# SonyResearch/micro_diffusion

Measured on AMD Instinct MI355X. Metric: training images/sec (global batch 2048) MicroDiT-XL/2 256-res mask=0.75, higher is better.
Workload: dtype bf16; 1 GPU; MicroDiT_XL_2 res_256_pretrain.yaml mask=0.75, full step = 2 microbatches x 1024 fwd+bwd + grad exchange + clip 0.25 + AdamW; global_batch=2048, microbatch=1024, parallelism=dp1, grad_exchange=none (single rank)

## Files before the change

### micro_diffusion_amd/csrc/gemm.hip

```cpp
#include "md_common.h"
#include "gemm_common.h"
#include <stdlib.h>

namespace {

constexpr int BM = 128, BN = 128;
constexpr int PITCH_KC = (BKT + 8) * 2;
constexpr int PITCH_KS = (BM + 32) * 2;
constexpr int TILE_BYTES = (BM * PITCH_KC > BKT * PITCH_KS) ? BM * PITCH_KC : BKT * PITCH_KS;
constexpr int SLAB_PITCH = 68;
constexpr int SLAB_FLOATS = 32 * SLAB_PITCH;
static_assert(4 * SLAB_FLOATS * 4 <= 2 * TILE_BYTES, "epilogue slab must fit in the staging LDS");

typedef __attribute__((address_space(3))) s16x4 lds_s16x4;

__device__ __forceinline__ bf16x4 lds_tr_read(const unsigned char* p) {
    s16x4 v = __builtin_amdgcn_ds_read_tr16_b64_v4i16((lds_s16x4*)(p));
    U64 t;
    t.s = v;
    return t.h;
}

__device__ __forceinline__ void tile_coords(int bid, int nwg, int ntn, int group_n, int& tm, int& tn) {
    const int q = nwg >> 3, r = nwg & 7, xcd = bid & 7, j = bid >> 3;
// ... 366 lines not shown
    long long* const tl = static_cast<long long*>(p.timeline);
    timeline_stamp(tl, 0);
    const int64_t m0 = (int64_t)tile_m * TM;
    const int64_t n0 = (int64_t)tile_n * TN;
    const int batch = blockIdx.y / p.ksplit;
    const int split = blockIdx.y % p.ksplit;
    const bf16* A = reinterpret_cast<const bf16*>(p.A) + (int64_t)batch * p.sA;
    const bf16* B = reinterpret_cast<const bf16*>(p.B) + (int64_t)batch * p.sB;
    const int64_t ntk = (p.K + BKT - 1) / BKT;
    const int64_t tps = (ntk + p.ksplit - 1) / p.ksplit;
    const int64_t kbeg = (int64_t)split * tps * BKT;
    int64_t kend = kbeg + tps * BKT;
    if (kend > p.K) kend = p.K;
    const int nt = kbeg < kend ? (int)((kend - kbeg + BKT - 1) / BKT) : 0;

    f32x16 acc[MI][2];
#pragma unroll
    for (int i = 0; i < MI; ++i)
#pragma unroll
        for (int j = 0; j < 2; ++j)
#pragma unroll
            for (int r = 0; r < 16; ++r) acc[i][j][r] = 0.f;

    const unsigned lds0 = (unsigned)(uintptr_t)(lds_void_t*)smem;
    if (nt > 0) {
        dma_tile<AKC, TM>(smem, A, p.lda, m0, p.M, kbeg, kend, wave, lane);
        dma_tile<BKC, TN>(smem + ATILE, B, p.ldb, n0, p.N, kbeg, kend, wave, lane);
    }
    bf16x8 fa[2][MI], fb[2][2];
    for (int t = 0; t < nt; ++t) {
        const int cur = t & 1;
        const bool more = t + 1 < nt;
        const int64_t k0 = kbeg + (int64_t)(t + 1) * BKT;
        unsigned char* nb = smem + (cur ^ 1) * BUF;
        if (PACED) {
            asm volatile("s_waitcnt vmcnt(0)" ::: "memory");
            __builtin_amdgcn_s_barrier();
        } else {
            if (more) {
                dma_tile<AKC, TM>(nb, A, p.lda, m0, p.M, k0, kend, wave, lane);
                dma_tile<BKC, TN>(nb + ATILE, B, p.ldb, n0, p.N, k0, kend, wave, lane);
                asm volatile("s_waitcnt vmcnt(8)" ::: "memory");
            } else {
                asm volatile("s_waitcnt vmcnt(0)" ::: "memory");
            }
            __builtin_amdgcn_s_barrier();
        }
        if (t == 0) timeline_stamp(tl, 1);
        const unsigned sA = lds0 + cur * BUF, sB = sA + ATILE;
#pragma unroll
        for (int i = 0; i < MI; ++i) fa[0][i] = dma_frag<AKC, TM>(sA, wm * (MI * 32) + i * 32, 0, lane);
#pragma unroll
        for (int j = 0; j < 2; ++j) fb[0][j] = dma_frag<BKC, TN>(sB, wn * 64 + j * 32, 0, lane);
        asm volatile("s_waitcnt lgkmcnt(0)" ::: "memory");
#pragma unroll
        for (int ks = 0; ks < BKT / 16; ++ks) {
            const int cb = ks & 1, nx = cb ^ 1;
            if (PACED && more) {
                dma_tile<AKC, TM>(nb, A, p.lda, m0, p.M, k0, kend, wave, lane, ks, ks + 1);
                dma_tile<BKC, TN>(nb + ATILE, B, p.ldb, n0, p.N, k0, kend, wave, lane, ks, ks + 1);
            }
            if (ks + 1 < BKT / 16) {
#pragma unroll
                for (int i = 0; i < MI; ++i) fa[nx][i] = dma_frag<AKC, TM>(sA, wm * (MI * 32) + i * 32, ks + 1, lane);
#pragma unroll
                for (int j = 0; j < 2; ++j) fb[nx][j] = dma_frag<BKC, TN>(sB, wn * 64 + j * 32, ks + 1, lane);
            }
            __builtin_amdgcn_sched_barrier(0);
#pragma unroll
            for (int i = 0; i < MI; ++i)
#pragma unroll
                for (int j = 0; j < 2; ++j)
                    acc[i][j] = __builtin_amdgcn_mfma_f32_32x32x16_bf16(fa[cb][i], fb[cb][j], acc[i][j], 0, 0, 0);
            __builtin_amdgcn_sched_barrier(0);
            if (ks + 1 < BKT / 16) asm volatile("s_waitcnt lgkmcnt(0)" ::: "memory");
            __builtin_amdgcn_sched_barrier(0);
        }
        if (!PACED) __builtin_amdgcn_s_barrier();
    }
    if (PACED) __builtin_amdgcn_s_barrier();
    timeline_stamp(tl, 2);
    gemm_epilogue<MI>(p, acc, smem, m0 + wm * (MI * 32), n0 + wn * 64, batch, split, wave, lane);
    timeline_finish(tl);
}

__device__ __forceinline__ float4 nt_ld4(const float* p) {
    const f32x4 v = __builtin_nontemporal_load(reinterpret_cast<const f32x4*>(p));
    return make_float4(v[0], v[1], v[2], v[3]);
}
__global__ __launch_bounds__(256) void splitk_reduce_kernel(const float* ws, float* out, int64_t M, int64_t N, int64_t ldo,
                                                            int64_t sOut, int ksplit, int batch, int accumulate, int64_t slice) {
    const int64_t n4 = N / 4, per = M * n4, total = per * batch;
    for (int64_t i = (int64_t)blockIdx.x * 256 + threadIdx.x; i < total; i += (int64_t)gridDim.x * 256) {
        const int64_t b = i / per, r = i % per, m = r / n4, c = (r % n4) * 4;
        const float* src = ws + (b * ksplit) * slice + m * N + c;
        float4 acc = make_float4(0.f, 0.f, 0.f, 0.f);
        int s = 0;
        for (; s + 4 <= ksplit; s += 4) {
            const float4 v0 = nt_ld4(src + (int64_t)s * slice), v1 = nt_ld4(src + (int64_t)(s + 1) * slice);
            const float4 v2 = nt_ld4(src + (int64_t)(s + 2) * slice), v3 = nt_ld4(src + (int64_t)(s + 3) * slice);
            acc.x += (v0.x + v1.x) + (v2.x + v3.x); acc.y += (v0.y + v1.y) + (v2.y + v3.y);
            acc.z += (v0.z + v1.z) + (v2.z + v3.z); acc.w += (v0.w + v1.w) + (v2.w + v3.w);
        }
        for (; s < ksplit; ++s) {
            const float4 v = nt_ld4(src + (int64_t)s * slice);
            acc.x += v.x; acc.y += v.y; acc.z += v.z; acc.w += v.w;
        }
        if (accumulate == 2) {
            bf16x4 o;
            o[0] = f2bf(acc.x); o[1] = f2bf(acc.y); o[2] = f2bf(acc.z); o[3] = f2bf(acc.w);
            st_bf16x4(reinterpret_cast<bf16*>(out) + b * sOut + m * ldo + c, o);
            continue;
        }
        float* dst = out + b * sOut + m * ldo + c;
        if (accumulate) {
            const float4 o = *reinterpret_cast<const float4*>(dst);
            acc.x += o.x; acc.y += o.y; acc.z += o.z; acc.w += o.w;
        }
        *reinterpret_cast<float4*>(dst) = acc;
    }
}

}

extern "C" int md_splitk_reduce(const float* ws, float* out, int64_t M, int64_t N, int64_t ldo, int64_t sOut, int32_t ksplit,
                                int32_t batch, int32_t accumulate, hipStream_t stream) {
    if (!ws || !out || M <= 0 || N <= 0 || N % 4 || ldo % 4 || ksplit <= 0 || batch <= 0 || accumulate < 0 || accumulate > 2) return MD_BAD_ARG;
    int64_t grid = (M * (N / 4) * batch + 255) / 256;
    if (grid > 16384) grid = 16384;
    hipLaunchKernelGGL(splitk_reduce_kernel, dim3((unsigned)grid), dim3(256), 0, stream, ws, out, M, N, ldo, sOut, ksplit, batch,
                       accumulate, M * N);
    MD_LAUNCH_CHECK();
    return 0;
}

extern "C" int md_splitk_reduce_flat(const float* ws, float* out, int64_t n, int64_t slice_stride, int32_t ksplit, int32_t accumulate,
                                     hipStream_t stream) {
    if (!ws || !out || n <= 0 || n % 4 || slice_stride < n || slice_stride % 4 || ksplit <= 0 || accumulate < 0 || accumulate > 2) return MD_BAD_ARG;
    int64_t grid = (n / 4 + 255) / 256;
    if (grid > 16384) grid = 16384;
    hipLaunchKernelGGL(splitk_reduce_kernel, dim3((unsigned)grid), dim3(256), 0, stream, ws, out, (int64_t)1, n, n, (int64_t)0, ksplit, 1,
                       accumulate, slice_stride);
    MD_LAUNCH_CHECK();
    return 0;
}

static bool md_gemm_w4_fills(int64_t tiles, int cu_limit) {
    if (!(cu_limit > 0 && cu_limit < 256)) return true;
    if (tiles <= cu_limit) return false;
    const int64_t rounds = (tiles + cu_limit - 1) / cu_limit;
    return tiles * 100 >= rounds * cu_limit * 92;
}

extern "C" int md_gemm_bf16(const md_gemm_args* a_in, hipStream_t stream) {
    if (!a_in) return MD_BAD_ARG;
    md_gemm_args a_copy = *a_in;
    const md_gemm_args* a = &a_copy;
    if (a->problems) {
        if (!a->C || a->K <= 0 || a->ksplit <= 0 || a->mode != MD_EPI_STORE_F32 || a->sSplit <= 0 || !md_gemm_pp_eligible(a)) return MD_BAD_ARG;
        if (a->variant != MD_GEMM_AUTO && a->variant != MD_GEMM_PP256 && a->variant != MD_GEMM_W4) return MD_NOT_ELIGIBLE;
        if (a->variant == MD_GEMM_W4 && !md_gemm_w4_eligible(a)) return MD_NOT_ELIGIBLE;
        bool w4 = a->variant == MD_GEMM_W4;
        if (a->variant == MD_GEMM_AUTO && md_gemm_w4_eligible(a) && !getenv("MD_GEMM_NO_W4") && !getenv("MD_GEMM_NO_W4_TN")) {
            int64_t t = 0;
            for (int i = 0; i < a->n_problems; ++i) t += ((a->problems[i].M + 255) / 256) * ((a->problems[i].N + 255) / 256);
            w4 = md_gemm_w4_fills(t * a->ksplit, a->cu_limit);
        }
        if (a->chosen_variant) *a->chosen_variant = w4 ? MD_GEMM_W4 : MD_GEMM_PP256;
        return w4 ? md_gemm_w4_launch(a, stream) : md_gemm_pp_launch(a, stream);
    }
    if (!a->A || !a->B || !a->C) return MD_BAD_ARG;
    if (a->M <= 0 || a->N <= 0 || a->K <= 0 || a->batch <= 0 || a->ksplit <= 0) return MD_BAD_ARG;
    if (a->lda % 8 || a->ldb % 8) return MD_BAD_ARG;
    if ((a->mode == MD_EPI_STORE_BF16 || a->mode == MD_EPI_RESIDUAL || a->mode == MD_EPI_DACT || a->mode == MD_EPI_SWIGLU_BWD) ? (a->ldc % 8) : (a->ldc % 4))
        return MD_BAD_ARG;
    if (a->C2 && a->ldc2 % 8) return MD_BAD_ARG;
    if (a->ksplit > 1 && !(a->mode == MD_EPI_ATOMIC_F32 || (a->mode == MD_EPI_STORE_F32 && a->sSplit > 0))) return MD_BAD_ARG;
    if (a->mode == MD_EPI_RESIDUAL && (!a->res || (a->gate && a->rows_per_sample <= 0))) return MD_BAD_ARG;
    if (a->mode == MD_EPI_DACT && !a->aux) return MD_BAD_ARG;
    if (a->mode < MD_EPI_STORE_BF16 || a->mode > MD_EPI_SWIGLU_BWD) return MD_BAD_ARG;
    if (a->mode == MD_EPI_SWIGLU_BWD) {
        if (!a->aux || a->ldaux % 8) return MD_BAD_ARG;
        if (a->variant != MD_GEMM_AUTO && a->variant != MD_GEMM_W4) return MD_NOT_ELIGIBLE;
        if (!md_gemm_w4_eligible(a) || (a->cu_limit > 0 && a->cu_limit < 256) || getenv("MD_GEMM_NO_W4")) return MD_NOT_ELIGIBLE;
        a_copy.variant = MD_GEMM_W4;
    }
    if (a->dact_cached && (a->act != MD_ACT_GELU_ERF || !(a->mode == MD_EPI_DACT || (a->mode == MD_EPI_STORE_BF16 && a->C2)))) return MD_BAD_ARG;
    const int64_t tiles256 = ((a->M + 255) / 256) * ((a->N + 255) / 256) * (int64_t)a->batch * a->ksplit;
    const int64_t kspan = (a->K + a->ksplit - 1) / a->ksplit;
    int variant = a->variant;
    if (variant < MD_GEMM_AUTO || variant > MD_GEMM_W4) return MD_BAD_ARG;
    if (variant == MD_GEMM_PP256 && !md_gemm_pp_eligible(a)) return MD_NOT_ELIGIBLE;
    if (variant == MD_GEMM_W4 && !md_gemm_w4_eligible(a)) return MD_NOT_ELIGIBLE;
    if ((a->A_list || a->B_list) && !(a->A_list && a->B_list && md_gemm_pp_eligible(a))) return MD_BAD_ARG;
    if (a->A_list) variant = MD_GEMM_PP256;
    if (variant == MD_GEMM_AUTO) {
        const char* w4min = getenv("MD_GEMM_W4_MIN_TILES");
        if (md_gemm_w4_eligible(a) && tiles256 >= (w4min ? atoi(w4min) : 192) && md_gemm_w4_fills(tiles256, a->cu_limit) && !getenv("MD_GEMM_NO_W4") &&
            (a->a_kcontig || !getenv("MD_GEMM_NO_W4_TN")))
            variant = MD_GEMM_W4;
        else if (md_gemm_pp_eligible(a) && tiles256 >= 192)
            variant = MD_GEMM_PP256;
        else if (!a->a_kcontig && !a->b_kcontig && kspan >= 2048 && tiles256 >= 128)
            variant = MD_GEMM_PACED256;
        else if (a->K >= 1024 && tiles256 >= 224 && tiles256 <= 256)
            variant = MD_GEMM_PACED256;
        else if (kspan > 2048 && tiles256 >= 240 && (tiles256 % 256 == 0 || tiles256 % 256 >= 160 || tiles256 >= 2048))
            variant = MD_GEMM_PACED256;
        else if (a->a_kcontig && a->K <= 2048)
            variant = MD_GEMM_REG128;
        else
            variant = ((!a->a_kcontig && !a->b_kcontig) || a->K < 1024) ? MD_GEMM_REG128 : MD_GEMM_DMA128;
    }
    const int TMv = variant >= MD_GEMM_PACED256 ? 256 : 128;
    if (a->raster_group_n <= 0) {
        const int64_t ntn_ = (a->N + TMv - 1) / TMv;
        int64_t g = (2 << 20) / (TMv * kspan * 2);
        if (variant >= MD_GEMM_PP256 && g < 4) g = 4;
        if (g < 1) g = 1;
        if (g > ntn_) g = ntn_;
        a_copy.raster_group_n = (int)g;
    }
    if (a->chosen_variant) *a->chosen_variant = variant;
    if (variant == MD_GEMM_W4) return md_gemm_w4_launch(a, stream);
    if (variant >= MD_GEMM_PP256) return md_gemm_pp_launch(a, stream);
    const int64_t tiles = ((a->M + TMv - 1) / TMv) * ((a->N + TMv - 1) / TMv);
    dim3 grid((unsigned)tiles, (unsigned)(a->batch * a->ksplit), 1);
#define LAUNCH(KERN, THREADS, ...)                                                                                          \
    do {                                                                                                                   \
        if (a->a_kcontig && a->b_kcontig) hipLaunchKernelGGL((KERN<1, 1 __VA_ARGS__>), grid, dim3(THREADS), 0, stream, *a);       \
        else if (a->a_kcontig && !a->b_kcontig) hipLaunchKernelGGL((KERN<1, 0 __VA_ARGS__>), grid, dim3(THREADS), 0, stream, *a); \
        else if (!a->a_kcontig && a->b_kcontig) hipLaunchKernelGGL((KERN<0, 1 __VA_ARGS__>), grid, dim3(THREADS), 0, stream, *a); \
        else hipLaunchKernelGGL((KERN<0, 0 __VA_ARGS__>), grid, dim3(THREADS), 0, stream, *a);                                     \
    } while (0)
#define COMMA ,
    if (variant == MD_GEMM_REG128) LAUNCH(gemm_bf16_kernel, 256, );
    else if (variant == MD_GEMM_DMA128) LAUNCH(gemm_bf16_dma_kernel, 256, COMMA 2 COMMA 2 COMMA 2);
    else LAUNCH(gemm_bf16_dma_kernel, 512, COMMA 2 COMMA 4 COMMA 4 COMMA true);
#undef COMMA
#undef LAUNCH
    MD_LAUNCH_CHECK();
    return 0;
}
```

### micro_diffusion_amd/csrc/gemm_w4.hip

```cpp
#include "gemm_pp_common.h"

namespace {

struct W4Addr {
    unsigned adA[8];
    unsigned adB[8];
    unsigned aofs[8], bofs[8];
    unsigned ldsw;
};

#ifndef W4_ACC_INC
#define W4_ACC_INC "gemm_w4_acc.inc"
#endif
#include W4_ACC_INC

constexpr int W4_BUF = 32768;
constexpr int W4_BREG = 65536;
constexpr int W4_SLAB = 8192;

constexpr bool w4_is_dact(int epi) { return epi == PP_E_DACT_GELU || epi == PP_E_DACT_MUL || epi == PP_E_DACT_SWIGLU; }



typedef unsigned w4_u32x2 __attribute__((ext_vector_type(2), may_alias));
typedef unsigned w4_u32x4 __attribute__((ext_vector_type(4), may_alias));

struct W4Tile {
    int m0, n0, batch;
    int mlim, nlim;
    char* cbase;
    char* c2base;
    const char* opbase;
    const char* gbase;
};

struct W4EpiLane {
    unsigned wr[8];
    unsigned rd[4];
    unsigned oc, oc2, oo, og;
    int rg, c8;
};
struct W4Ops {
    uint4 v[4];
    uint4 gq;
    uint4 v2[4];
};

template <int EPI>
__device__ __forceinline__ void w4_epi_lane(const md_gemm_args& p, const W4Tile& et, int wcol, int lane_in, W4EpiLane& L) {
    int lane = lane_in;
    asm volatile("" : "+v"(lane));
    const int r = lane & 15, g = lane >> 4;
#pragma unroll
    for (int j = 0; j < 8; ++j) L.wr[j] = (unsigned)(r * 256 + ((32 * j + 8 * g) ^ (r << 4)));
#pragma unroll
    for (int t = 0; t < 4; ++t) L.rd[t] = (unsigned)((4 * t + g) * 256 + ((16 * r) ^ ((4 * t + g) << 4)));
    L.rg = g;
    L.c8 = r * 8;
    const int cc = wcol + r * 8 < et.nlim ? r * 8 : 0;
    L.oc = (unsigned)(g * (int)p.ldc + r * 8) * 2u;
    L.oc2 = (unsigned)(g * (int)p.ldc2 + r * 8) * 2u;
    L.oo = (unsigned)(g * (int)(EPI == PP_E_RES ? p.ldr : p.ldaux) + cc) * 2u;
    L.og = (unsigned)cc * 2u;
}

struct W4Rows {
    char* c;
    char* c2;
    const char* op;
    int64_t sc, sc2, so;
};

template <int EPI, bool INTERIOR>
__device__ __forceinline__ void w4_epi_req(const md_gemm_args& p, const W4Tile& et, const W4EpiLane& L, const char* oprow, int row0, int wcol, uint4& dst) {
    if (INTERIOR) {
        dst = *reinterpret_cast<const uint4*>(oprow + L.oo);
    } else if constexpr (EPI == PP_E_DACT_SWIGLU) {
        dst = make_uint4(0u, 0u, 0u, 0u);
    } else {
        const int64_t ldo = EPI == PP_E_RES ? p.ldr : p.ldaux;
        const int row = row0 + L.rg < et.mlim - 1 ? row0 + L.rg : et.mlim - 1;
        dst = *reinterpret_cast<const uint4*>(et.opbase + ((int64_t)row * ldo + wcol) * 2 + L.og);
    }
}
template <int EPI, int I>
__device__ __forceinline__ void w4_epi_gate(const md_gemm_args& p, const PPPlan& w, const W4Tile& et, const W4EpiLane& L, int wrow, int wcol, uint4& gq) {
    gq = make_uint4(0x3f803f80u, 0x3f803f80u, 0x3f803f80u, 0x3f803f80u);
    if (et.gbase) {
        int r0 = et.m0 + wrow + 16 * I;
        r0 = r0 < w.M - 1 ? r0 : w.M - 1;
        const unsigned srow = w.rps_shift >= 0 ? (unsigned)r0 >> w.rps_shift : (unsigned)r0 / (unsigned)p.rows_per_sample;
        gq = *reinterpret_cast<const uint4*>(et.gbase + ((int64_t)srow * p.ldg + wcol) * 2 + L.og);
    }
}

template <int I>
__device__ __forceinline__ void w4_epi_write(unsigned char* slab, const W4EpiLane& L) {
    unsigned char* half = slab + (I & 1) * 4096;
#pragma unroll
    for (int jh = 0; jh < 2; ++jh) {
        float a[16];
        if (jh == 0) w4_acc_read16<I, 0>(a);
        else w4_acc_read16<I, 1>(a);
#pragma unroll
        for (int q = 0; q < 4; ++q) {
            const w4_u32x2 v = {cvt_pk_bf16(a[4 * q], a[4 * q + 1]), cvt_pk_bf16(a[4 * q + 2], a[4 * q + 3])};
            *reinterpret_cast<w4_u32x2*>(half + L.wr[4 * jh + q]) = v;
        }
    }
}

template <int EPI, int I, bool INTERIOR>
__device__ __forceinline__ void w4_epi_store(const md_gemm_args& p, const PPPlan& w, const W4Tile& et, const W4EpiLane& L, int wrow, int wcol,
                                             const w4_u32x4 (&Tv)[4], W4Ops& ops, W4Rows& R) {
#pragma unroll
    for (int t = 0; t < 4; ++t) {
        const uint4 T = make_uint4(Tv[t].x, Tv[t].y, Tv[t].z, Tv[t].w);
        const int row0 = wrow + 16 * I + 4 * t;
        const bool ok = INTERIOR || (wcol + L.c8 < et.nlim && row0 + L.rg < et.mlim);
        char* const crow = R.c;
        uint4 out = T;
        if constexpr (EPI == PP_E_BF16 || EPI == PP_E_RES || EPI == PP_E_BF16_GELU) {
            if (et.c2base && ok) *reinterpret_cast<uint4*>(R.c2 + L.oc2) = T;
        }
        if constexpr (EPI == PP_E_BF16_GELU) {
            float v[8];
            unpack8(T, v);
#pragma unroll
            for (int e = 0; e < 8; e += 2) {
                const f32x2 g2 = gelu_erf_2(f32x2{v[e], v[e + 1]});
                v[e] = g2.x;
                v[e + 1] = g2.y;
            }
            out = make_uint4(cvt_pk_bf16(v[0], v[1]), cvt_pk_bf16(v[2], v[3]), cvt_pk_bf16(v[4], v[5]), cvt_pk_bf16(v[6], v[7]));
        } else if constexpr (EPI == PP_E_BF16_GELU_D) {
            float v[8], dv[8];
            unpack8(T, v);
#pragma unroll
            for (int e = 0; e < 8; e += 2) {
                f32x2 g2, d2;
                gelu_dgelu_erf_2(f32x2{v[e], v[e + 1]}, g2, d2);
                v[e] = g2.x;
                v[e + 1] = g2.y;
                dv[e] = d2.x;
                dv[e + 1] = d2.y;
            }
            out = make_uint4(cvt_pk_bf16(v[0], v[1]), cvt_pk_bf16(v[2], v[3]), cvt_pk_bf16(v[4], v[5]), cvt_pk_bf16(v[6], v[7]));
            if (et.c2base && ok)
                *reinterpret_cast<uint4*>(R.c2 + L.oc2) =
                    make_uint4(cvt_pk_bf16(dv[0], dv[1]), cvt_pk_bf16(dv[2], dv[3]), cvt_pk_bf16(dv[4], dv[5]), cvt_pk_bf16(dv[6], dv[7]));
        } else if constexpr (EPI == PP_E_RES) {
            const uint4 gq = ops.gq;
            const unsigned lw[4] = {T.x, T.y, T.z, T.w}, rw[4] = {ops.v[t].x, ops.v[t].y, ops.v[t].z, ops.v[t].w}, gw[4] = {gq.x, gq.y, gq.z, gq.w};
            unsigned ow[4];
#pragma unroll
            for (int h = 0; h < 4; ++h) {
                const float y0 = __uint_as_float(lw[h] << 16), y1 = __uint_as_float(lw[h] & 0xffff0000u);
                const float r0 = __uint_as_float(rw[h] << 16), r1 = __uint_as_float(rw[h] & 0xffff0000u);
                const float g0 = __uint_as_float(gw[h] << 16), g1 = __uint_as_float(gw[h] & 0xffff0000u);
                ow[h] = cvt_pk_bf16(r0 + g0 * y0, r1 + g1 * y1);
            }
            out = make_uint4(ow[0], ow[1], ow[2], ow[3]);
        } else if constexpr (EPI == PP_E_DACT_MUL) {
            float v[8], ax[8];
            unpack8(T, v);
            unpack8(ops.v[t], ax);
#pragma unroll
            for (int e = 0; e < 8; ++e) v[e] *= ax[e];
            out = make_uint4(cvt_pk_bf16(v[0], v[1]), cvt_pk_bf16(v[2], v[3]), cvt_pk_bf16(v[4], v[5]), cvt_pk_bf16(v[6], v[7]));
        } else if constexpr (EPI == PP_E_DACT_SWIGLU) {
            float g[8], x1[8], x2[8], o2[8];
            unpack8(T, g);
            unpack8(ops.v[t], x1);
            unpack8(ops.v2[t], x2);
#pragma unroll
            for (int e = 0; e < 8; ++e) {
                const float sg = __builtin_amdgcn_rcpf(1.f + __builtin_amdgcn_exp2f(x1[e] * -1.4426950408889634f));
                const float sl = x1[e] * sg;
                o2[e] = g[e] * sl;
                g[e] = g[e] * x2[e] * (sg + sl * (1.f - sg));
            }
            out = make_uint4(cvt_pk_bf16(g[0], g[1]), cvt_pk_bf16(g[2], g[3]), cvt_pk_bf16(g[4], g[5]), cvt_pk_bf16(g[6], g[7]));
            if (ok) *reinterpret_cast<uint4*>(crow + L.oc + 2 * (int64_t)p.N) =
                make_uint4(cvt_pk_bf16(o2[0], o2[1]), cvt_pk_bf16(o2[2], o2[3]), cvt_pk_bf16(o2[4], o2[5]), cvt_pk_bf16(o2[6], o2[7]));
        } else if constexpr (EPI == PP_E_DACT_GELU) {
            float v[8], ax[8];
            unpack8(T, v);
            unpack8(ops.v[t], ax);
#pragma unroll
            for (int e = 0; e < 8; e += 2) {
                const f32x2 d = dgelu_erf_2(f32x2{ax[e], ax[e + 1]});
                v[e] *= d.x;
                v[e + 1] *= d.y;
            }
            out = make_uint4(cvt_pk_bf16(v[0], v[1]), cvt_pk_bf16(v[2], v[3]), cvt_pk_bf16(v[4], v[5]), cvt_pk_bf16(v[6], v[7]));
        }
#ifdef W4_X_NOSTORE
        asm volatile("" : : "v"(out.x), "v"(out.y), "v"(out.z), "v"(out.w));
#else
        if (ok) *reinterpret_cast<uint4*>(crow + L.oc) = out;
#endif
        if constexpr ((EPI == PP_E_RES || w4_is_dact(EPI)) && I < 7) {
            w4_epi_req<EPI, INTERIOR>(p, et, L, R.op, row0 + 16, wcol, ops.v[t]);
            if constexpr (EPI == PP_E_DACT_SWIGLU) w4_epi_req<EPI, INTERIOR>(p, et, L, R.op + 2 * (int64_t)p.N, row0 + 16, wcol, ops.v2[t]);
        }
        R.c += R.sc;
        R.c2 += R.sc2;
        R.op += R.so;
    }
    if constexpr (EPI == PP_E_RES && I < 7) w4_epi_gate<EPI, I + 1>(p, w, et, L, wrow, wcol, ops.gq);
}

template <int I>
__device__ __forceinline__ void w4_epi_read(unsigned char* slab, const W4EpiLane& L, w4_u32x4 (&Tv)[4]) {
    unsigned char* half = slab + (I & 1) * 4096;
#pragma unroll
    for (int t = 0; t < 4; ++t) Tv[t] = *reinterpret_cast<const w4_u32x4*>(half + L.rd[t]);
}

template <int EPI, bool INTERIOR>
__device__ __forceinline__ void w4_epilogue(const md_gemm_args& p, const PPPlan& w, const W4Tile& et, unsigned char* slab, int wrow, int wcol, int lane) {
    W4EpiLane L;
    w4_epi_lane<EPI>(p, et, wcol, lane, L);
    W4Ops ops;
    W4Rows R;
    const int64_t ldo = EPI == PP_E_RES ? p.ldr : p.ldaux;
    R.sc = 8 * p.ldc;
    R.sc2 = 8 * p.ldc2;
    R.so = 8 * ldo;
    R.c = et.cbase + ((int64_t)wrow * p.ldc + wcol) * 2;
    R.c2 = et.c2base ? et.c2base + ((int64_t)wrow * p.ldc2 + wcol) * 2 : nullptr;
    R.op = nullptr;
    if constexpr (EPI == PP_E_RES || w4_is_dact(EPI)) {
        R.op = et.opbase + ((int64_t)wrow * ldo + wcol) * 2;
#pragma unroll
        for (int t = 0; t < 4; ++t) {
            w4_epi_req<EPI, INTERIOR>(p, et, L, R.op, wrow + 4 * t, wcol, ops.v[t]);
            if constexpr (EPI == PP_E_DACT_SWIGLU) w4_epi_req<EPI, INTERIOR>(p, et, L, R.op + 2 * (int64_t)p.N, wrow + 4 * t, wcol, ops.v2[t]);
            R.op += R.so;
        }
        if constexpr (EPI == PP_E_RES) w4_epi_gate<EPI, 0>(p, w, et, L, wrow, wcol, ops.gq);
    }
    w4_u32x4 Tv[4];
    w4_epi_write<0>(slab, L);
#define W4_EPI_STEP(I)                                                                                                  \
    w4_epi_read<I>(slab, L, Tv);                                                                                        \
    if constexpr ((I) < 7) w4_epi_write<((I) < 7 ? (I) + 1 : 7)>(slab, L);                                               \
    if constexpr ((I) == 0) asm volatile("s_waitcnt vmcnt(0)" ::: "memory");                                             \
    w4_epi_store<EPI, I, INTERIOR>(p, w, et, L, wrow, wcol, Tv, ops, R);
    W4_EPI_STEP(0) W4_EPI_STEP(1) W4_EPI_STEP(2) W4_EPI_STEP(3) W4_EPI_STEP(4) W4_EPI_STEP(5) W4_EPI_STEP(6) W4_EPI_STEP(7)
#undef W4_EPI_STEP
}

__device__ __forceinline__ void w4_epilogue_f32(float* tile, int64_t ldc, int wrow, int wcol, int lane_in) {
    int lane = lane_in;
    asm volatile("" : "+v"(lane));
    float* const p0 = tile + (int64_t)(wrow + (lane & 15)) * ldc + wcol + 4 * (lane >> 4);
    asm volatile("s_waitcnt vmcnt(0)" ::: "memory");
#define W4_F32_STEP(I, JH)                                                                                               \
    {                                                                                                                    \
        float a[16];                                                                                                     \
        w4_acc_read16<I, JH>(a);                                                                                         \
        float* const pr = p0 + (int64_t)(16 * (I)) * ldc + 64 * (JH);                                                    \
        _Pragma("unroll") for (int q = 0; q < 4; ++q)                                                                    \
            *reinterpret_cast<float4*>(pr + 16 * q) = make_float4(a[4 * q], a[4 * q + 1], a[4 * q + 2], a[4 * q + 3]);   \
    }
    W4_F32_STEP(0, 0) W4_F32_STEP(0, 1) W4_F32_STEP(1, 0) W4_F32_STEP(1, 1) W4_F32_STEP(2, 0) W4_F32_STEP(2, 1) W4_F32_STEP(3, 0) W4_F32_STEP(3, 1)
    W4_F32_STEP(4, 0) W4_F32_STEP(4, 1) W4_F32_STEP(5, 0) W4_F32_STEP(5, 1) W4_F32_STEP(6, 0) W4_F32_STEP(6, 1) W4_F32_STEP(7, 0) W4_F32_STEP(7, 1)
#undef W4_F32_STEP
}

template <int AKC, int BKC, int EPI>
__global__ __launch_bounds__(256) __attribute__((amdgpu_num_vgpr(144))) void gemm_bf16_w4_kernel(md_gemm_args p, PPPlan w) {
    __shared__ __attribute__((aligned(1024))) unsigned char smem[2 * W4_BREG + 4 * W4_SLAB];
    const int tid = threadIdx.x, lane = tid & 63;
    const int wave = __builtin_amdgcn_readfirstlane(tid >> 6);
    const int wr = wave >> 1, wc = wave & 1;

    int w_first, w_stride, w_count;
    {
        const int G = gridDim.x, x = blockIdx.x & 7, j = blockIdx.x >> 3;
        const int q = w.total >> 3, r = w.total & 7;
        const int lo = x < r ? x * (q + 1) : r * (q + 1) + (x - r) * q;
        const int cnt = q + (x < r ? 1 : 0);
        w_stride = (G - x + 7) >> 3;
        w_first = lo + j;
        w_count = j < cnt ? (int)((unsigned)(cnt - j + w_stride - 1) / (unsigned)w_stride) : 0;
    }
    if (w_count == 0) return;
    const int pairs = w_count * (w.nk >> 1);

    const unsigned lds0 = (unsigned)(uintptr_t)(lds_void_t*)smem;
    W4Addr ad;
    {
        const int ra = wr * 128 + (lane & 15), rb = wc * 128 + (lane & 15);
#pragma unroll
        for (int ks = 0; ks < 2; ++ks) {
            if (AKC) ad.adA[ks] = lds0 + (unsigned)(ra * 128 + ((((4 * ks + (lane >> 4)) ^ (ra >> 1)) & 7) << 4));
            if (BKC) ad.adB[ks] = lds0 + (unsigned)(W4_BREG + rb * 128 + ((((4 * ks + (lane >> 4)) ^ (rb >> 1)) & 7) << 4));
        }
        if (AKC) {
#pragma unroll
            for (int i = 2; i < 8; ++i) ad.adA[i] = 0;
        } else {
            const int li = lane & 15, g = lane >> 4;
            const int kk = 8 * g + (li >> 2);
            const int swz = ((kk & 3) << 1) | (((kk >> 3) & 1) << 3);
#pragma unroll
            for (int i = 0; i < 8; ++i) {
                const int col = wr * 128 + 16 * i + 4 * (li & 3);
                ad.adA[i] = lds0 + (unsigned)(kk * 512 + ((((col >> 3) ^ swz) & 31) << 4) + ((col >> 2) & 1) * 8);
            }
        }
        if (!BKC) {
            const int li = lane & 15, g = lane >> 4;
            const int kk = 8 * g + (li >> 2);
            const int swz = ((kk & 3) << 1) | (((kk >> 3) & 1) << 3);
#pragma unroll
            for (int j = 0; j < 8; ++j) {
                const int col = wc * 128 + 16 * j + 4 * (li & 3);
                ad.adB[j] = lds0 + (unsigned)(W4_BREG + kk * 512 + ((((col >> 3) ^ swz) & 31) << 4) + ((col >> 2) & 1) * 8);
            }
        } else {
#pragma unroll
            for (int j = 2; j < 8; ++j) ad.adB[j] = 0;
        }
    }
    ad.ldsw = lds0 + (unsigned)wave * 1024u;

    int s_n = 0, s_kt = 0, s_koffA = 0, s_koffB = 0;
    int kstepA = AKC ? BKT * 2 : BKT * w.lda * 2;
    int kstepB = BKC ? BKT * 2 : BKT * w.ldb * 2;
    constexpr bool GROUPABLE = !AKC && !BKC && EPI == PP_E_F32;
    u32x4 rA, rB;
    auto stager_open = [&](int n) {
        int m0, n0, batch, split;
        if (GROUPABLE && w.nprob) {
            int q;
            work_decode_grouped(w, w_first + n * w_stride, q, m0, n0, split);
            const PPProblem& pr = w.prob[q];
            const int sw = (tid >> 5) & 3;
#pragma unroll
            for (int x = 0; x < 8; ++x) {
                const int c8 = ((tid & 31) ^ ((sw << 1) | ((x & 1) << 3))) * 8;
                const int kr = x * 8 + (tid >> 5);
                ad.aofs[x] = (unsigned)(kr * pr.lda + c8) * 2u;
                ad.bofs[x] = (unsigned)(kr * pr.ldb + c8) * 2u;
            }
            kstepA = BKT * pr.lda * 2;
            kstepB = BKT * pr.ldb * 2;
            const int64_t kb = (int64_t)split * w.kspan;
            const uint64_t ua = (uint64_t)(uintptr_t)(reinterpret_cast<const bf16*>(pr.A) + kb * pr.lda + m0);
            const uint64_t ub = (uint64_t)(uintptr_t)(reinterpret_cast<const bf16*>(pr.B) + kb * pr.ldb + n0);
            rA = u32x4{(unsigned)ua, (unsigned)(ua >> 32) & 0xffffu, 0xffffffffu, 0x00020000u};
            rB = u32x4{(unsigned)ub, (unsigned)(ub >> 32) & 0xffffu, 0xffffffffu, 0x00020000u};
            s_koffA = 0;
            s_koffB = 0;
            return;
        }
        work_decode(w, w_first + n * w_stride, m0, n0, batch, split);
        const int c = ((tid & 7) ^ ((tid >> 4) & 7)) * 8;
#pragma unroll
        for (int x = 0; x < 8; ++x) {
            const int row = x * 32 + (tid >> 3);
            if (AKC) {
                int ga = m0 + row;
                ga = (ga < w.M ? ga : w.M - 1) - m0;
                ad.aofs[x] = (unsigned)(ga * w.lda + c) * 2u;
            } else {
                int gc = m0 + ((tid & 31) ^ ((((tid >> 5) & 3) << 1) | ((x & 1) << 3))) * 8;
                const int last = (w.M - 1) & ~7;
                gc = (gc < last ? gc : last) - m0;
                ad.aofs[x] = (unsigned)((x * 8 + (tid >> 5)) * w.lda + gc) * 2u;
            }
            if (BKC) {
                int gb = n0 + row;
                gb = (gb < w.N ? gb : w.N - 1) - n0;
                ad.bofs[x] = (unsigned)(gb * w.ldb + c) * 2u;
            } else {
                int gc = n0 + ((tid & 31) ^ ((((tid >> 5) & 3) << 1) | ((x & 1) << 3))) * 8;
                const int last = (w.N - 1) & ~7;
                gc = (gc < last ? gc : last) - n0;
                ad.bofs[x] = (unsigned)((x * 8 + (tid >> 5)) * w.ldb + gc) * 2u;
            }
        }
        const int64_t kbeg = (int64_t)split * w.kspan;
        const bf16* pa = reinterpret_cast<const bf16*>(p.A) + (int64_t)batch * p.sA + (AKC ? (int64_t)m0 * w.lda + kbeg : kbeg * w.lda + m0);
        const bf16* pb = reinterpret_cast<const bf16*>(p.B) + (int64_t)batch * p.sB + (BKC ? (int64_t)n0 * w.ldb + kbeg : kbeg * w.ldb + n0);
        const uint64_t ua = (uint64_t)(uintptr_t)pa, ub = (uint64_t)(uintptr_t)pb;
        rA = u32x4{(unsigned)ua, (unsigned)(ua >> 32) & 0xffffu, 0xffffffffu, 0x00020000u};
        rB = u32x4{(unsigned)ub, (unsigned)(ub >> 32) & 0xffffu, 0xffffffffu, 0x00020000u};
        s_koffA = 0;
        s_koffB = 0;
    };
    auto stager_pair_done = [&]() {
        s_kt += 2;
        if (s_kt == w.nk) {
            s_kt = 0;
            if (s_n + 1 < w_count) ++s_n;
            stager_open(s_n);
        }
    };
    stager_open(0);
    w4_prologue<AKC, BKC>(ad, rA, rB, 0, 0, kstepA, kstepB);
    s_koffA = 2 * kstepA;
    s_koffB = 2 * kstepB;
    stager_pair_done();
    w4_first_reads<AKC, BKC>(ad);

    int c_n = 0, c_kt = 0;
#define W4_KTILE(BUF, FRESH)                                                                                            \
    do {                                                                                                                \
        w4_h0<AKC, BKC, BUF, FRESH>(ad, rA, rB, s_koffA, s_koffB);                                                      \
        w4_h1<AKC, BKC, BUF, FRESH>(ad, rA, rB, s_koffA, s_koffB);                                                      \
        w4_h2<AKC, BKC, BUF, FRESH>(ad, rA, rB, s_koffA, s_koffB);                                                      \
        s_koffA += kstepA;                                                                                              \
        s_koffB += kstepB;                                                                                              \
        w4_h3<AKC, BKC, BUF>(ad);                                                                                       \
    } while (0)

    for (int it = 0; it < pairs; ++it) {
        if (c_kt == 0) W4_KTILE(0, true);
        else W4_KTILE(0, false);
        W4_KTILE(1, false);
        stager_pair_done();
        c_kt += 2;
        if (c_kt == w.nk) {
            if constexpr (EPI == PP_E_F32) {
                int m0, n0, batch = 0, split;
                float* tile;
                int64_t ldc;
                if (GROUPABLE && w.nprob) {
                    int q;
                    work_decode_grouped(w, w_first + c_n * w_stride, q, m0, n0, split);
                    const PPProblem& pr = w.prob[q];
                    ldc = pr.N;
                    tile = reinterpret_cast<float*>(p.C) + (int64_t)split * p.sSplit + pr.c_off + (int64_t)m0 * ldc + n0;
                } else {
                    work_decode(w, w_first + c_n * w_stride, m0, n0, batch, split);
                    ldc = p.ldc;
                    tile = reinterpret_cast<float*>(p.C) + (int64_t)batch * p.sC + (int64_t)split * p.sSplit + (int64_t)m0 * ldc + n0;
                }
                asm volatile("s_nop 15\n\ts_nop 15");
                w4_epilogue_f32(tile, ldc, wr * 128, wc * 128, lane);
                c_kt = 0;
                ++c_n;
                continue;
            }
            W4Tile et;
            int split;
            work_decode(w, w_first + c_n * w_stride, et.m0, et.n0, et.batch, split);
            et.mlim = w.M - et.m0;
            et.nlim = w.N - et.n0;
            et.cbase = reinterpret_cast<char*>(p.C) + ((int64_t)et.batch * p.sC + (int64_t)et.m0 * p.ldc + et.n0) * 2;
            et.c2base = (!w4_is_dact(EPI) && p.C2) ? reinterpret_cast<char*>(p.C2) + ((int64_t)et.batch * p.sC2 + (int64_t)et.m0 * p.ldc2 + et.n0) * 2 : nullptr;
            et.opbase = EPI == PP_E_RES   ? reinterpret_cast<const char*>(p.res) + ((int64_t)et.m0 * p.ldr + et.n0) * 2
                        : w4_is_dact(EPI) ? reinterpret_cast<const char*>(p.aux) + ((int64_t)et.batch * p.sAux + (int64_t)et.m0 * p.ldaux + et.n0) * 2
                                          : nullptr;
            et.gbase = (EPI == PP_E_RES && p.gate) ? reinterpret_cast<const char*>(p.gate) + (size_t)et.n0 * 2 : nullptr;
            asm volatile("s_nop 15\n\ts_nop 15");
#ifndef W4_X_NOEPI
            unsigned char* const slab = smem + 2 * W4_BREG + wave * W4_SLAB;
            if (et.mlim >= PT && et.nlim >= PT) w4_epilogue<EPI, true>(p, w, et, slab, wr * 128, wc * 128, lane);
            else w4_epilogue<EPI, false>(p, w, et, slab, wr * 128, wc * 128, lane);
#else
            asm volatile("s_waitcnt vmcnt(0)" ::: "memory");
#endif
            c_kt = 0;
            ++c_n;
        }
    }
    asm volatile("s_waitcnt vmcnt(0)" ::: "memory");
}

}

static bool w4_instantiated(int akc, int bkc, int epi) {
    if (!akc) return !bkc && epi == PP_E_F32;
    if (bkc) return epi == PP_E_BF16 || epi == PP_E_RES || epi == PP_E_DACT_GELU || epi == PP_E_DACT_MUL;
    return epi == PP_E_BF16 || epi == PP_E_BF16_GELU || epi == PP_E_BF16_GELU_D || epi == PP_E_RES || epi == PP_E_DACT_SWIGLU;
}

bool md_gemm_w4_eligible(const md_gemm_args* a) {
    const int epi = md_gemm_pp_epi_kind(a);
    if (epi < 0 || !w4_instantiated(a->a_kcontig, a->b_kcontig, epi)) return false;
    if (!md_gemm_pp_shape_ok(a, epi)) return false;
    if (epi == PP_E_DACT_SWIGLU && (!a->aux || a->batch != 1 || a->ldaux < 2 * a->N || a->ldc < 2 * a->N)) return false;
    if (a->A_list || a->B_list || a->timeline) return false;
    if (a->bias || a->alpha != 1.f) return false;
    const int64_t kspan = a->K / a->ksplit;
    if (epi == PP_E_F32) {
        if (a->ksplit > 1 && a->sSplit <= 0) return false;
        if (a->problems) {
            for (int i = 0; i < a->n_problems; ++i) {
                const md_gemm_problem& s = a->problems[i];
                if (s.M % PT || s.N % PT || kspan * (s.lda > s.ldb ? s.lda : s.ldb) >= ((int64_t)1 << 30)) return false;
            }
            return true;
        }
        if (a->M % PT || a->N % PT || a->ldc % 4) return false;
        return kspan * (a->lda > a->ldb ? a->lda : a->ldb) < ((int64_t)1 << 30);
    }
    if (a->ksplit != 1 || a->problems) return false;
    if (!a->b_kcontig && (a->K * a->ldb >= (int64_t)1 << 30)) return false;
    return true;
}

int md_gemm_w4_launch(const md_gemm_args* a, hipStream_t stream) {
    PPPlan w;
    if (!md_gemm_pp_plan(a, &w)) return MD_BAD_ARG;
    const int cus = (a->cu_limit > 0 && a->cu_limit < NUM_CU) ? a->cu_limit : NUM_CU;
    const unsigned G = (unsigned)(w.total < cus ? w.total : cus);
    if (a->tail_used) *a->tail_used = 0;
    const int epi = md_gemm_pp_epi_kind(a);
    const dim3 grid(G, 1, 1), block(256);
#define W4_LAUNCH(AK, BK, E) hipLaunchKernelGGL((gemm_bf16_w4_kernel<AK, BK, E>), grid, block, 0, stream, *a, w)
    if (!a->a_kcontig) {
        W4_LAUNCH(0, 0, PP_E_F32);
    } else if (a->b_kcontig) {
        if (epi == PP_E_BF16) W4_LAUNCH(1, 1, PP_E_BF16);
        else if (epi == PP_E_RES) W4_LAUNCH(1, 1, PP_E_RES);
        else if (epi == PP_E_DACT_MUL) W4_LAUNCH(1, 1, PP_E_DACT_MUL);
        else W4_LAUNCH(1, 1, PP_E_DACT_GELU);
    } else {
        if (epi == PP_E_BF16) W4_LAUNCH(1, 0, PP_E_BF16);
        else if (epi == PP_E_BF16_GELU) W4_LAUNCH(1, 0, PP_E_BF16_GELU);
        else if (epi == PP_E_BF16_GELU_D) W4_LAUNCH(1, 0, PP_E_BF16_GELU_D);
        else if (epi == PP_E_DACT_SWIGLU) W4_LAUNCH(1, 0, PP_E_DACT_SWIGLU);
        else W4_LAUNCH(1, 0, PP_E_RES);
    }
#undef W4_LAUNCH
    MD_LAUNCH_CHECK();
    return 0;
}
```

Baseline: 2806 images/sec.

## Deepen W4 epilogue operand prefetch ring and cache GEMM env lookups

```diff
diff --git a/micro_diffusion_amd/csrc/gemm.hip b/micro_diffusion_amd/csrc/gemm.hip
--- a/micro_diffusion_amd/csrc/gemm.hip
+++ b/micro_diffusion_amd/csrc/gemm.hip
@@ -542,8 +542,21 @@
     return tiles * 100 >= rounds * cu_limit * 92;
 }
 
+struct GemmEnv {
+    bool no_w4, no_w4_tn;
+    int w4_min_tiles;
+};
+static const GemmEnv& md_gemm_env() {
+    static const GemmEnv e = [] {
+        const char* w4min = getenv("MD_GEMM_W4_MIN_TILES");
+        return GemmEnv{getenv("MD_GEMM_NO_W4") != nullptr, getenv("MD_GEMM_NO_W4_TN") != nullptr, w4min ? atoi(w4min) : 192};
+    }();
+    return e;
+}
+
 extern "C" int md_gemm_bf16(const md_gemm_args* a_in, hipStream_t stream) {
     if (!a_in) return MD_BAD_ARG;
+    const GemmEnv& env = md_gemm_env();
     md_gemm_args a_copy = *a_in;
     const md_gemm_args* a = &a_copy;
     if (a->problems) {
@@ -551,7 +564,7 @@
         if (a->variant != MD_GEMM_AUTO && a->variant != MD_GEMM_PP256 && a->variant != MD_GEMM_W4) return MD_NOT_ELIGIBLE;
         if (a->variant == MD_GEMM_W4 && !md_gemm_w4_eligible(a)) return MD_NOT_ELIGIBLE;
         bool w4 = a->variant == MD_GEMM_W4;
-        if (a->variant == MD_GEMM_AUTO && md_gemm_w4_eligible(a) && !getenv("MD_GEMM_NO_W4") && !getenv("MD_GEMM_NO_W4_TN")) {
+        if (a->variant == MD_GEMM_AUTO && md_gemm_w4_eligible(a) && !env.no_w4 && !env.no_w4_tn) {
             int64_t t = 0;
             for (int i = 0; i < a->n_problems; ++i) t += ((a->problems[i].M + 255) / 256) * ((a->problems[i].N + 255) / 256);
             w4 = md_gemm_w4_fills(t * a->ksplit, a->cu_limit);
@@ -572,7 +585,7 @@
     if (a->mode == MD_EPI_SWIGLU_BWD) {
         if (!a->aux || a->ldaux % 8) return MD_BAD_ARG;
         if (a->variant != MD_GEMM_AUTO && a->variant != MD_GEMM_W4) return MD_NOT_ELIGIBLE;
-        if (!md_gemm_w4_eligible(a) || (a->cu_limit > 0 && a->cu_limit < 256) || getenv("MD_GEMM_NO_W4")) return MD_NOT_ELIGIBLE;
+        if (!md_gemm_w4_eligible(a) || (a->cu_limit > 0 && a->cu_limit < 256) || env.no_w4) return MD_NOT_ELIGIBLE;
         a_copy.variant = MD_GEMM_W4;
     }
     if (a->dact_cached && (a->act != MD_ACT_GELU_ERF || !(a->mode == MD_EPI_DACT || (a->mode == MD_EPI_STORE_BF16 && a->C2)))) return MD_BAD_ARG;
@@ -585,9 +598,8 @@
     if ((a->A_list || a->B_list) && !(a->A_list && a->B_list && md_gemm_pp_eligible(a))) return MD_BAD_ARG;
     if (a->A_list) variant = MD_GEMM_PP256;
     if (variant == MD_GEMM_AUTO) {
-        const char* w4min = getenv("MD_GEMM_W4_MIN_TILES");
-        if (md_gemm_w4_eligible(a) && tiles256 >= (w4min ? atoi(w4min) : 192) && md_gemm_w4_fills(tiles256, a->cu_limit) && !getenv("MD_GEMM_NO_W4") &&
-            (a->a_kcontig || !getenv("MD_GEMM_NO_W4_TN")))
+        if (md_gemm_w4_eligible(a) && tiles256 >= env.w4_min_tiles && md_gemm_w4_fills(tiles256, a->cu_limit) && !env.no_w4 &&
+            (a->a_kcontig || !env.no_w4_tn))
             variant = MD_GEMM_W4;
         else if (md_gemm_pp_eligible(a) && tiles256 >= 192)
             variant = MD_GEMM_PP256;
diff --git a/micro_diffusion_amd/csrc/gemm_w4.hip b/micro_diffusion_amd/csrc/gemm_w4.hip
--- a/micro_diffusion_amd/csrc/gemm_w4.hip
+++ b/micro_diffusion_amd/csrc/gemm_w4.hip
@@ -37,19 +37,21 @@
 struct W4EpiLane {
     unsigned wr[8];
     unsigned rd[4];
-    unsigned oc, oc2, oo, og;
+    unsigned oc, oc2, oo;
     int rg, c8;
 };
+constexpr bool w4_reads_operand(int epi) { return epi == PP_E_RES || w4_is_dact(epi); }
+constexpr int w4_ring(int epi, int bkc) { return epi == PP_E_DACT_SWIGLU ? 6 : (epi == PP_E_RES && !bkc) ? 5 : 8; }
 struct W4Ops {
-    uint4 v[4];
-    uint4 gq;
-    uint4 v2[4];
+    uint4 v[8];
+    uint4 gq[2];
+    uint4 v2[8];
 };
 
 template <int EPI>
-__device__ __forceinline__ void w4_epi_lane(const md_gemm_args& p, const W4Tile& et, int wcol, int lane_in, W4EpiLane& L) {
-    int lane = lane_in;
-    asm volatile("" : "+v"(lane));
+__device__ __forceinline__ void w4_epi_lane(const md_gemm_args& p, W4EpiLane& L) {
+    int lane;
+    asm volatile("v_mbcnt_lo_u32_b32 %0, -1, 0\n\tv_mbcnt_hi_u32_b32 %0, -1, %0" : "=v"(lane));
     const int r = lane & 15, g = lane >> 4;
 #pragma unroll
     for (int j = 0; j < 8; ++j) L.wr[j] = (unsigned)(r * 256 + ((32 * j + 8 * g) ^ (r << 4)));
@@ -57,11 +59,9 @@
     for (int t = 0; t < 4; ++t) L.rd[t] = (unsigned)((4 * t + g) * 256 + ((16 * r) ^ ((4 * t + g) << 4)));
     L.rg = g;
     L.c8 = r * 8;
-    const int cc = wcol + r * 8 < et.nlim ? r * 8 : 0;
     L.oc = (unsigned)(g * (int)p.ldc + r * 8) * 2u;
     L.oc2 = (unsigned)(g * (int)p.ldc2 + r * 8) * 2u;
-    L.oo = (unsigned)(g * (int)(EPI == PP_E_RES ? p.ldr : p.ldaux) + cc) * 2u;
-    L.og = (unsigned)cc * 2u;
+    L.oo = (unsigned)(g * (int)(EPI == PP_E_RES ? p.ldr : p.ldaux) + r * 8) * 2u;
 }
 
 struct W4Rows {
@@ -71,17 +71,11 @@
     int64_t sc, sc2, so;
 };
 
-template <int EPI, bool INTERIOR>
-__device__ __forceinline__ void w4_epi_req(const md_gemm_args& p, const W4Tile& et, const W4EpiLane& L, const char* oprow, int row0, int wcol, uint4& dst) {
-    if (INTERIOR) {
-        dst = *reinterpret_cast<const uint4*>(oprow + L.oo);
-    } else if constexpr (EPI == PP_E_DACT_SWIGLU) {
-        dst = make_uint4(0u, 0u, 0u, 0u);
-    } else {
-        const int64_t ldo = EPI == PP_E_RES ? p.ldr : p.ldaux;
-        const int row = row0 + L.rg < et.mlim - 1 ? row0 + L.rg : et.mlim - 1;
-        dst = *reinterpret_cast<const uint4*>(et.opbase + ((int64_t)row * ldo + wcol) * 2 + L.og);
-    }
+template <int EPI>
+__device__ __forceinline__ void w4_epi_req(const md_gemm_args& p, const W4EpiLane& L, W4Rows& R, W4Ops& ops, int slot) {
+    ops.v[slot] = *reinterpret_cast<const uint4*>(R.op + L.oo);
+    if constexpr (EPI == PP_E_DACT_SWIGLU) ops.v2[slot] = *reinterpret_cast<const uint4*>(R.op + 2 * (int64_t)p.N + L.oo);
+    R.op += R.so;
 }
 template <int EPI, int I>
 __device__ __forceinline__ void w4_epi_gate(const md_gemm_args& p, const PPPlan& w, const W4Tile& et, const W4EpiLane& L, int wrow, int wcol, uint4& gq) {
@@ -90,7 +84,9 @@
         int r0 = et.m0 + wrow + 16 * I;
         r0 = r0 < w.M - 1 ? r0 : w.M - 1;
         const unsigned srow = w.rps_shift >= 0 ? (unsigned)r0 >> w.rps_shift : (unsigned)r0 / (unsigned)p.rows_per_sample;
-        gq = *reinterpret_cast<const uint4*>(et.gbase + ((int64_t)srow * p.ldg + wcol) * 2 + L.og);
+        unsigned og;
+        asm volatile("v_mbcnt_lo_u32_b32 %0, -1, 0\n\tv_mbcnt_hi_u32_b32 %0, -1, %0" : "=v"(og));
+        gq = *reinterpret_cast<const uint4*>(et.gbase + ((int64_t)srow * p.ldg + wcol) * 2 + (og & 15u) * 16u);
     }
 }
 
@@ -110,17 +106,19 @@
     }
 }
 
-template <int EPI, int I, bool INTERIOR>
+template <int EPI, int I, bool INTERIOR, int RING>
 __device__ __forceinline__ void w4_epi_store(const md_gemm_args& p, const PPPlan& w, const W4Tile& et, const W4EpiLane& L, int wrow, int wcol,
                                              const w4_u32x4 (&Tv)[4], W4Ops& ops, W4Rows& R) {
+    static_assert(INTERIOR || !w4_reads_operand(EPI), "operand-reading epilogues: interior tiles only");
 #pragma unroll
     for (int t = 0; t < 4; ++t) {
+        const int slot = (4 * I + t) % RING;
         const uint4 T = make_uint4(Tv[t].x, Tv[t].y, Tv[t].z, Tv[t].w);
         const int row0 = wrow + 16 * I + 4 * t;
         const bool ok = INTERIOR || (wcol + L.c8 < et.nlim && row0 + L.rg < et.mlim);
         char* const crow = R.c;
         uint4 out = T;
-        if constexpr (EPI == PP_E_BF16 || EPI == PP_E_RES || EPI == PP_E_BF16_GELU) {
+        if constexpr (EPI == PP_E_BF16 || EPI == PP_E_BF16_GELU) {
             if (et.c2base && ok) *reinterpret_cast<uint4*>(R.c2 + L.oc2) = T;
         }
         if constexpr (EPI == PP_E_BF16_GELU) {
@@ -150,8 +148,8 @@
                 *reinterpret_cast<uint4*>(R.c2 + L.oc2) =
                     make_uint4(cvt_pk_bf16(dv[0], dv[1]), cvt_pk_bf16(dv[2], dv[3]), cvt_pk_bf16(dv[4], dv[5]), cvt_pk_bf16(dv[6], dv[7]));
         } else if constexpr (EPI == PP_E_RES) {
-            const uint4 gq = ops.gq;
-            const unsigned lw[4] = {T.x, T.y, T.z, T.w}, rw[4] = {ops.v[t].x, ops.v[t].y, ops.v[t].z, ops.v[t].w}, gw[4] = {gq.x, gq.y, gq.z, gq.w};
+            const uint4 gq = ops.gq[I & 1], rq = ops.v[slot];
+            const unsigned lw[4] = {T.x, T.y, T.z, T.w}, rw[4] = {rq.x, rq.y, rq.z, rq.w}, gw[4] = {gq.x, gq.y, gq.z, gq.w};
             unsigned ow[4];
 #pragma unroll
             for (int h = 0; h < 4; ++h) {
@@ -164,29 +162,29 @@
         } else if constexpr (EPI == PP_E_DACT_MUL) {
             float v[8], ax[8];
             unpack8(T, v);
-            unpack8(ops.v[t], ax);
+            unpack8(ops.v[slot], ax);
 #pragma unroll
             for (int e = 0; e < 8; ++e) v[e] *= ax[e];
             out = make_uint4(cvt_pk_bf16(v[0], v[1]), cvt_pk_bf16(v[2], v[3]), cvt_pk_bf16(v[4], v[5]), cvt_pk_bf16(v[6], v[7]));
         } else if constexpr (EPI == PP_E_DACT_SWIGLU) {
             float g[8], x1[8], x2[8], o2[8];
             unpack8(T, g);
-            unpack8(ops.v[t], x1);
-            unpack8(ops.v2[t], x2);
+            unpack8(ops.v[slot], x1);
+            unpack8(ops.v2[slot], x2);
 #pragma unroll
             for (int e = 0; e < 8; ++e) {
                 const float sg = __builtin_amdgcn_rcpf(1.f + __builtin_amdgcn_exp2f(x1[e] * -1.4426950408889634f));
                 const float sl = x1[e] * sg;
                 o2[e] = g[e] * sl;
-                g[e] = g[e] * x2[e] * (sg + sl * (1.f - sg));
+                g[e] = g[e] * x2[e] * __builtin_fmaf(sl, 1.f - sg, sg);
             }
             out = make_uint4(cvt_pk_bf16(g[0], g[1]), cvt_pk_bf16(g[2], g[3]), cvt_pk_bf16(g[4], g[5]), cvt_pk_bf16(g[6], g[7]));
-            if (ok) *reinterpret_cast<uint4*>(crow + L.oc + 2 * (int64_t)p.N) =
+            *reinterpret_cast<uint4*>(crow + L.oc + 2 * (int64_t)p.N) =
                 make_uint4(cvt_pk_bf16(o2[0], o2[1]), cvt_pk_bf16(o2[2], o2[3]), cvt_pk_bf16(o2[4], o2[5]), cvt_pk_bf16(o2[6], o2[7]));
         } else if constexpr (EPI == PP_E_DACT_GELU) {
             float v[8], ax[8];
             unpack8(T, v);
-            unpack8(ops.v[t], ax);
+            unpack8(ops.v[slot], ax);
 #pragma unroll
             for (int e = 0; e < 8; e += 2) {
                 const f32x2 d = dgelu_erf_2(f32x2{ax[e], ax[e + 1]});
@@ -194,21 +192,24 @@
                 v[e + 1] *= d.y;
             }
             out = make_uint4(cvt_pk_bf16(v[0], v[1]), cvt_pk_bf16(v[2], v[3]), cvt_pk_bf16(v[4], v[5]), cvt_pk_bf16(v[6], v[7]));
+        }
+        if constexpr (w4_reads_operand(EPI)) {
+            if (4 * I + t + RING < 32) w4_epi_req<EPI>(p, L, R, ops, slot);
+            if constexpr (EPI == PP_E_RES && I + 2 < 8) {
+                if (t == 3) w4_epi_gate<EPI, I + 2>(p, w, et, L, wrow, wcol, ops.gq[I & 1]);
+            }
+            if constexpr (EPI == PP_E_RES) {
+                if (et.c2base) *reinterpret_cast<uint4*>(R.c2 + L.oc2) = T;
+            }
         }
 #ifdef W4_X_NOSTORE
         asm volatile("" : : "v"(out.x), "v"(out.y), "v"(out.z), "v"(out.w));
 #else
         if (ok) *reinterpret_cast<uint4*>(crow + L.oc) = out;
 #endif
-        if constexpr ((EPI == PP_E_RES || w4_is_dact(EPI)) && I < 7) {
-            w4_epi_req<EPI, INTERIOR>(p, et, L, R.op, row0 + 16, wcol, ops.v[t]);
-            if constexpr (EPI == PP_E_DACT_SWIGLU) w4_epi_req<EPI, INTERIOR>(p, et, L, R.op + 2 * (int64_t)p.N, row0 + 16, wcol, ops.v2[t]);
-        }
         R.c += R.sc;
         R.c2 += R.sc2;
-        R.op += R.so;
-    }
-    if constexpr (EPI == PP_E_RES && I < 7) w4_epi_gate<EPI, I + 1>(p, w, et, L, wrow, wcol, ops.gq);
+    }
 }
 
 template <int I>
@@ -218,10 +219,10 @@
     for (int t = 0; t < 4; ++t) Tv[t] = *reinterpret_cast<const w4_u32x4*>(half + L.rd[t]);
 }
 
-template <int EPI, bool INTERIOR>
-__device__ __forceinline__ void w4_epilogue(const md_gemm_args& p, const PPPlan& w, const W4Tile& et, unsigned char* slab, int wrow, int wcol, int lane) {
+template <int EPI, bool INTERIOR, int RING>
+__device__ __forceinline__ void w4_epilogue(const md_gemm_args& p, const PPPlan& w, const W4Tile& et, unsigned char* slab, int wrow, int wcol) {
     W4EpiLane L;
-    w4_epi_lane<EPI>(p, et, wcol, lane, L);
+    w4_epi_lane<EPI>(p, L);
     W4Ops ops;
     W4Rows R;
     const int64_t ldo = EPI == PP_E_RES ? p.ldr : p.ldaux;
@@ -231,15 +232,14 @@
     R.c = et.cbase + ((int64_t)wrow * p.ldc + wcol) * 2;
     R.c2 = et.c2base ? et.c2base + ((int64_t)wrow * p.ldc2 + wcol) * 2 : nullptr;
     R.op = nullptr;
-    if constexpr (EPI == PP_E_RES || w4_is_dact(EPI)) {
+    if constexpr (w4_reads_operand(EPI)) {
         R.op = et.opbase + ((int64_t)wrow * ldo + wcol) * 2;
 #pragma unroll
-        for (int t = 0; t < 4; ++t) {
-            w4_epi_req<EPI, INTERIOR>(p, et, L, R.op, wrow + 4 * t, wcol, ops.v[t]);
-            if constexpr (EPI == PP_E_DACT_SWIGLU) w4_epi_req<EPI, INTERIOR>(p, et, L, R.op + 2 * (int64_t)p.N, wrow + 4 * t, wcol, ops.v2[t]);
-            R.op += R.so;
-        }
-        if constexpr (EPI == PP_E_RES) w4_epi_gate<EPI, 0>(p, w, et, L, wrow, wcol, ops.gq);
+        for (int s = 0; s < RING; ++s) w4_epi_req<EPI>(p, L, R, ops, s);
+        if constexpr (EPI == PP_E_RES) {
+            w4_epi_gate<EPI, 0>(p, w, et, L, wrow, wcol, ops.gq[0]);
+            w4_epi_gate<EPI, 1>(p, w, et, L, wrow, wcol, ops.gq[1]);
+        }
     }
     w4_u32x4 Tv[4];
     w4_epi_write<0>(slab, L);
@@ -247,7 +247,7 @@
     w4_epi_read<I>(slab, L, Tv);                                                                                        \
     if constexpr ((I) < 7) w4_epi_write<((I) < 7 ? (I) + 1 : 7)>(slab, L);                                               \
     if constexpr ((I) == 0) asm volatile("s_waitcnt vmcnt(0)" ::: "memory");                                             \
-    w4_epi_store<EPI, I, INTERIOR>(p, w, et, L, wrow, wcol, Tv, ops, R);
+    w4_epi_store<EPI, I, INTERIOR, RING>(p, w, et, L, wrow, wcol, Tv, ops, R);
     W4_EPI_STEP(0) W4_EPI_STEP(1) W4_EPI_STEP(2) W4_EPI_STEP(3) W4_EPI_STEP(4) W4_EPI_STEP(5) W4_EPI_STEP(6) W4_EPI_STEP(7)
 #undef W4_EPI_STEP
 }
@@ -461,8 +461,8 @@
             asm volatile("s_nop 15\n\ts_nop 15");
 #ifndef W4_X_NOEPI
             unsigned char* const slab = smem + 2 * W4_BREG + wave * W4_SLAB;
-            if (et.mlim >= PT && et.nlim >= PT) w4_epilogue<EPI, true>(p, w, et, slab, wr * 128, wc * 128, lane);
-            else w4_epilogue<EPI, false>(p, w, et, slab, wr * 128, wc * 128, lane);
+            if (w4_reads_operand(EPI) || (et.mlim >= PT && et.nlim >= PT)) w4_epilogue<EPI, true, w4_ring(EPI, BKC)>(p, w, et, slab, wr * 128, wc * 128);
+            else if constexpr (!w4_reads_operand(EPI)) w4_epilogue<EPI, false, w4_ring(EPI, BKC)>(p, w, et, slab, wr * 128, wc * 128);
 #else
             asm volatile("s_waitcnt vmcnt(0)" ::: "memory");
 #endif
```

Result: no change. 2815 images/sec, median of 6 (+0.3%).
